# EMI-Group/evogp

Hardware: AMD Instinct MI355X
Metric: tree_evals_per_s (higher is better)
Workload: dtype f32; 1 GPU; BASELINE north_star / configs[2] shape: SymbolicRegression synthetic 10-var, GLOBAL pop=1000000 x 1024 datapoints, max_tree_len=64, funcs + - * /, one tree_SR_fitness pass over every rank's shard per step; global_pop=1000000, pop_per_gpu=1000000, datapoints=1024, var_len=10, max_tree_len=64, ranks=1, device_prewarm_calls=40

## Files before the change

evogp_amd/_lib.py:

```python
from __future__ import annotations

import ctypes as C
import os

_HERE = os.path.dirname(os.path.abspath(__file__))
LIB_PATH = os.environ.get("EVOGP_HIP_LIB") or os.path.join(_HERE, "lib", "libevogp_hip.so")

ABI_VERSION = 9

_vp = C.c_void_p
_u = C.c_uint
_i = C.c_int
_f = C.c_float

PROTOTYPES = {
    "evogp_hip_generate": [_u, _u, _u, _u, _u, _f, _f, _vp, _vp, _vp, _vp, _vp, _vp, _vp, _u, _vp],
    "evogp_hip_mutate": [_i, _i, _vp, _vp, _vp, _vp, _vp, _vp, _vp, _vp, _vp, _vp, _vp],
    "evogp_hip_crossover": [_i, _i, _i, _vp, _vp, _vp, _vp, _vp, _vp, _vp, _vp, _vp, _vp, _vp],
    "evogp_hip_evaluate": [_u, _u, _u, _u, _vp, _vp, _vp, _vp, _vp, _vp],
    "evogp_hip_sr_fitness": [_u, _u, _u, _u, _u, _i, _vp, _vp, _vp, _vp, _vp, _vp, _u, _vp],
    "evogp_hip_generate_masked": [_u, _u, _u, _u, _u, _f, _f, _vp, _vp, _vp, _vp, _vp, _vp, _vp, _u, _vp, _u, _vp],
    "evogp_hip_breed_default": [_i, _i, _i, _i, _vp, _vp, _vp, _vp, _vp, _u, _vp, _vp, _vp, _vp, _vp, _vp, _vp, _vp],
    "evogp_hip_breed_default_rows": [_i, _i, _i, _i, _vp, _vp, _vp, _vp, _vp, _u, _vp, _vp, _vp, _vp, _vp, _vp, _vp, _i, _i, _vp],
    "evogp_hip_breed_default_table": [_i, _i, _i, _i, _i, _vp, _vp, _vp, _vp, _vp, _u, _vp, _vp, _vp, _vp, _vp, _vp, _vp, _i, _i, _vp],
# ... 36 lines not shown
    "evogp_hip_tree_classes": [_u, _u, _vp, _vp, _vp, _vp, _vp, _vp, _vp],
    "evogp_hip_sr_linear_scaling": [_u, _u, _u, _u, _u, _vp, _vp, _vp, _vp, _vp, _vp, _vp, _vp],
    "evogp_hip_wrap_linear": [_u, _u, _u, _vp, _vp, _vp, _vp, _vp, _vp, _vp, _vp, _vp],
    "evogp_hip_tree_intervals": [_u, _u, _u, _vp, _vp, _vp, _vp, _vp, _vp, _vp, _vp, _vp],
    "evogp_hip_tree_derivative_intervals": [_u, _u, _u, _vp, _vp, _vp, _vp, _vp, _u, _vp, _vp, _vp, _vp, _vp, _vp, _vp, _vp],
}

DEBUG_PROTOTYPES = {
    "evogp_hip_timer_begin": [_vp],
    "evogp_hip_timer_end": [_vp, C.POINTER(C.c_float)],
    "evogp_hip_debug_set_stats": [_vp],
    "evogp_hip_debug_compile_batch": [_i],
    "evogp_hip_debug_long_compiler": [_i],
    "evogp_hip_debug_twins": [_i],
    "evogp_hip_debug_tc_fold": [_i],
    "evogp_hip_debug_profile": [_i],
    "evogp_hip_debug_profile_read": [C.POINTER(C.c_float), C.POINTER(C.c_int)],
    "evogp_hip_debug_tc_histogram": [_u, _vp, _i, _vp],
    "evogp_hip_debug_tc_nhandlers": [],
    "evogp_hip_debug_tc_program": [_u, _vp, _i],
    "evogp_hip_debug_forget_function_classes": [],
    "evogp_hip_debug_structural_mutate_given": [_i, _i, _i, _i, _i, _vp, _vp, _vp, _vp, _vp, _vp, _vp, _vp],
    "evogp_hip_debug_insert_mutate_given": [_i, _i, _i, _vp, _vp, _vp, _vp, _vp, _vp, _vp, _vp, _vp, _vp, _vp],
    "evogp_hip_debug_point_mutate_given": [_i, _i, _i, _i, _i, _i, _i, _i, _i, _vp, _vp, _vp, _vp, _vp, _vp, _vp, _vp, _vp, _vp, _vp, _vp, _vp, _vp],
    "evogp_hip_debug_lexicase": [_vp, _i],
    "evogp_hip_debug_pareto_rank": [_i],
}


def _load() -> C.CDLL:
# ... 34 lines not shown
```

evogp_amd/csrc/gen/gen_tc_asm.py:

```python
#!/usr/bin/env python3
import os
import sys

sys.path.insert(0, os.path.dirname(os.path.abspath(__file__)))
from ocml_bodies import BODIES
from pair_rows import Pairing, check as check_pairing

FORMS = ("SS", "SV", "VS", "SC", "CS", "VV", "VC", "CV")
SENTINEL_HEAVY = 0x7FC0FEED
OPS = ("add", "sub", "mul", "div")
UNARY = ("neg", "abs", "sin", "cos", "tan", "sqrt", "lsqrt", "exp", "log", "llog")
GBIN = ("ldiv", "max", "min", "lt", "gt", "le", "ge", "pow", "lpow")
GUN = ("zero", "sinh", "cosh", "tanh", "one", "rcp")
HEAVY_REGS = 24
SLOT = 256
DIVIP_REGS = 12
DIVIP = ("SS", "SC", "CS")
DIVR = ("SV", "VV", "CV")
NOPF_TWINS = tuple(f"{op}_{form}" for op in ("add", "sub", "mul") for form in FORMS) + ("push_c", "push_v") \
    + tuple(f"divip_{f}" for f in DIVIP) + tuple(f"divr_{f}" for f in DIVR)
NHF = 37 + 2 * len(UNARY) + 8 + 2 + 4 + len(DIVIP) + 1 + 1 + len(DIVR) + len(NOPF_TWINS) + 1


NOPF = False
SPLAT = False
FMA_LOSS = False
PKARITH = True
DIVABREAST = True
PKCONST = True
TRUST = True
DIVFIX = False
DIVRANGE = True
DIV_LO, DIV_HI = 0x28800000, 0x56800000
EARLYREC = True
L2WARM = True
KWARM_LINES = 4
# ... 99 lines not shown
        hid[f"{uop}_S"], hid[f"{uop}_V"] = 36 + 2 * u, 37 + 2 * u
    hid["next"] = 36 + 2 * len(UNARY)
    nh = hid["next"] + 1
    for f, form in enumerate(FORMS):
        hid[f"gbin_{form}"] = nh + f
    hid["gun_S"], hid["gun_V"], hid["if_sss"], hid["acc_s"], hid["mo_begin"], hid["end_mo"] = (nh + 8 + i for i in range(6))
    for i, form in enumerate(DIVIP):
        hid[f"divip_{form}"] = nh + 14 + i
    hid["end_cls"] = nh + 14 + len(DIVIP)
    hid["swap"] = nh + 14 + len(DIVIP) + 1
    for i, form in enumerate(DIVR):
        hid[f"divr_{form}"] = nh + 14 + len(DIVIP) + 2 + i
    for i, name in enumerate(NOPF_TWINS):
        hid[name + "_np"] = nh + 14 + len(DIVIP) + 2 + len(DIVR) + i
    hid["nan_tree"] = nh + 14 + len(DIVIP) + 2 + len(DIVR) + len(NOPF_TWINS)
    assert NHF == hid["nan_tree"] + 1 and 2 * NHF * SLOT <= 65536
    twin = [False]

    A_REC, A_WORK, A_TREES, A_DISP, A_START, A_TICK = NV - 1, NV - 2, NV - 3, NV - 4, NV - 5, NV - 6

    def tick_begin():
        if stats:
            a(f"s_memtime s[{T1}:{T2}]")
            a("s_waitcnt lgkmcnt(0)")
            a(f"v_mov_b32 v{A_TICK}, s{T1}")

    def tick_end(acc):
        if stats:
            a(f"s_memtime s[{T1}:{T2}]")
            a("s_waitcnt lgkmcnt(0)")
            a(f"v_sub_u32 v{A_TICK}, s{T1}, v{A_TICK}")
# ... 866 lines not shown
        for op in ("add", "sub", "mul"):
            for form in FORMS:
                arith(op, form, fl)
        push_c()
        push_v()
        divip_stubs()
        divr_stubs()
        twin[0] = False
        begin("nan_tree", fl)
        a("s_set_gpr_idx_off")
        a(f"s_mov_b32 s{T1}, 0x7fc00000")
        a(f"s_mov_b32 m0, s{sB}")
        a(f"s_bitset1_b64 s[{sOK}:{sOK + 1}], s{sB}")
        a(f"v_writelane_b32 v7, s{T1}, m0")
        a(f"s_branch {lab('next_tree')}")
    a(f".org {lab('hbase')}+{SLOT * 2 * NHF}")

    ALLREL = MODE["SRC0"] | MODE["SRC1"] | MODE["SRC2"] | MODE["DST"]
    for fl in (0, 1):
        for form in DIVIP:
            a(f"{lab(f'divip_body_{form}{fl}')}:")
            nops = 2 if form == "SS" else 1
            m0_stack(ALLREL, -nops * K)
            tb = S0 + nops * K
            tmp = [tb + i for i in range(DIVIP_REGS)]
            q, acc = tmp[4], tmp[0]
            if form == "SS":
                xs, ys = [S0 + K + k for k in range(K)], [S0 + k for k in range(K)]
            elif form == "CS":
                xs, ys = [f"s{sA}"] * K, [S0 + k for k in range(K)]
# ... 1202 lines not shown
```

evogp_amd/csrc/sr_tc.hip:

```cpp
#include "interp.hpp"
#include "launch.hpp"
#include "sr_params.hpp"
#include "tc_interp_k8.inc"
#include "tc_interp_k4.inc"
#include "tc_interp_k1.inc"

#include <atomic>
#include <cstddef>
#include <mutex>
#include <cstdio>
#include <vector>

namespace evogp {

struct TcCompileParams {
    const float *value;
    const int16_t *type;
    const int16_t *size;
    uint2 *prog;
    float *fitness;
    unsigned *marks;
    unsigned *zero_next;
    int pop, gp_len, var_len;
    uint32_t unary_mask;
// ... 2 lines not shown
    uint32_t rec;
    uint32_t overflow;
    int depth;
    int out_len;
    int nblocks;
    int rows;
    int general;
    int heavy_reserve;
    int div_reserve;
    int classify;
    uint32_t recip;
    int twins;
    int long_fast;
    int learn;
    int nan_trees;
};

__device__ inline uint32_t division_in_place(uint32_t id, int after, const TcCompileParams &p) {
    if (id < 24u || id >= 32u) return id;
    const uint32_t form = id - 24u;
    const uint32_t ip = form == 0u ? (uint32_t)EVOGP_TC_H_DIVIP_SS : form == 3u ? (uint32_t)EVOGP_TC_H_DIVIP_SC : form == 4u ? (uint32_t)EVOGP_TC_H_DIVIP_CS : 0u;
    if (ip == 0u) return id;
    const int before = after + (form == 0u ? 1 : 0);
    return before + p.div_reserve <= p.depth ? ip : id;
}

enum : int { TC_S = 0, TC_V = 1, TC_C = 2 };
constexpr int kMarkSampleBlocks = 64;
constexpr int kZeroRounds = 3;
static std::atomic<int> g_long_fast{-1};
static std::atomic<int> g_twins{-1};
static std::atomic<int> g_fold{-1};
static std::atomic<int> g_compile_batch{-2};
static int tc_nan_trees() {
    static const int env_fold = env_int("EVOGP_TC_FOLD", 2);
    const int fo = g_fold.load(std::memory_order_relaxed);
    return fo >= 0 ? fo : (env_fold < 0 || env_fold > 2 ? 2 : env_fold);
}
static_assert(kSentinelHeavy == 0x7FC0FEEDu, "gen/gen_tc_asm.py SENTINEL_HEAVY");

__device__ inline float fold_bin4_fast(int op, float x, float y) {
    return op == 0 ? x + y : op == 1 ? x - y : op == 2 ? x * y : (y == 0.0f ? __builtin_nanf("") : x / y);
}

__device__ inline uint32_t tc_word0(int id, int slot, uint32_t pf_bytes, uint32_t aux = 0u) {
    return ((pf_bytes >> 10) << 24) | ((aux & 0xFFu) << 16) | (uint32_t)(((slot & 1) * EVOGP_TC_NHANDLERS + id) * EVOGP_TC_SLOT);
}
// ... 260 lines not shown
    const int hf = seli(kept, totf - (inclf - deltaf), 0);
    if (any(hf > p.depth)) return p.gp_len > 64 && p.general ? TREE_GENERAL : TREE_HEAVY;
    const int dform = id - 24;
    const int ip = seli(dform == 0, (int)EVOGP_TC_H_DIVIP_SS, seli(dform == 3, (int)EVOGP_TC_H_DIVIP_SC, seli(dform == 4, (int)EVOGP_TC_H_DIVIP_CS, 0)));
    const bool inplace = (ip != 0) & (hf + (int)(dform == 0) + p.div_reserve <= p.depth);
    id = seli(inplace, ip, id);
    if (p.twins)
        id += seli(next_word_has_variable(p, keptmask, kept, !pushc & seli(isB, lV | rV, kind == 0), is_root), 0,
                   no_prefetch_delta(isB & !pushc & !divr & (opx < 3), pushc, inplace, divr & !pushc));
    if (kept) rec[slot] = make_uint2(tc_word0(id, slot, pf, aux), d1);
    if (lane == 0) rec[n] = make_uint2(tc_word0(EVOGP_TC_H_END, n, p.ydelta), 0u);
    return TREE_OK;
}


template <bool U0>
__device__ inline int compile_pack_arith(const TcCompileParams &p, char *rec0, uint32_t roff, unsigned long long inm, int lo, int len, int ty, int sz, float val, int lane) {
    typedef unsigned long long M;
    auto bperm = [](int v, int i4) -> int { return __builtin_amdgcn_ds_bpermute(i4, v); };
    auto next = [](int v) -> int { return __builtin_amdgcn_update_dpp(0, v, 0x130 , 0xf, 0xf, true); };
    auto B = [](bool c) -> M { return __builtin_amdgcn_ballot_w64(c); };
    auto L = [](M m) -> bool { return __builtin_amdgcn_inverse_ballot_w64(m); };
    auto seli = [](bool c, int x, int y) -> int { return c ? x : y; };
    auto selu = [](bool c, uint32_t x, uint32_t y) -> uint32_t { return c ? x : y; };
    auto self = [](bool c, float x, float y) -> float { return c ? x : y; };
    const M Min = inm;
    const int end = lo + len;
    asm volatile("" : "+v"(ty), "+v"(val));
    const uint32_t f = (uint32_t)val;
    const M MV = B(ty == T_VAR), MC = B(ty == T_CONST), MBf = B(ty == T_BFUNC);
    const uint32_t opu = f - (uint32_t)F_ADD;
    const M M4 = MBf & B(opu < 4u);
// ... 114 lines not shown
        cls = seg_any(Min & B(kind == 3)) ? TREE_HEAVY : seg_any(Min & B(kind == 5)) ? TREE_GENERAL : seg_any(Min & Msb) ? TREE_HEAVY
            : seg_any(Min & Mhigh) ? (p.gp_len > 64 && p.general ? TREE_GENERAL : TREE_HEAVY) : seg_any(Mlong) ? TREE_HEAVY : TREE_OK;
    }
    const M Mdivown = MB & ~Mpushc & ~Mdivr & B(opx == 3);
    const M Mss = Mdivown & B(form == 0), Msc = Mdivown & B(form == 3), Mcs = Mdivown & B(form == 4);
    const int ip = seli(L(Mss), (int)EVOGP_TC_H_DIVIP_SS, seli(L(Msc), (int)EVOGP_TC_H_DIVIP_SC, (int)EVOGP_TC_H_DIVIP_CS));
    const M Minpl = (Mss | Msc | Mcs) & B(hf + seli(L(Mss), 1, 0) + p.div_reserve <= p.depth);
    id = seli(L(Minpl), ip, id);
    if (p.twins) {
        const M Muses = ~Mpushc & ~MU & ((MB & (MlV | MrV)) | (~MB & MV));
        const M Uk = Mkept & Muses;
        const M nxt = (((~keptwave) + (Uk << 1)) & keptwave) | Mroot;
        id += seli(L(nxt), 0, no_prefetch_delta(L(MB & ~Mpushc & ~Mdivr & B(opx < 3)), L(Mpushc), L(Minpl), L(Mdivr & ~Mpushc)));
    }
    const M Mok = B(cls == TREE_OK);
    if (L(Mkept & Mok & ~Mpz)) *(uint2 *)(rec0 + (roff + (uint32_t)slot * 8u)) = make_uint2(tc_word0(id, slot, pf, aux), d1);
    if (L(Mroot)) {
        uint32_t skip = tc_word0(EVOGP_TC_H_SKIP, 0, 0u), nan_tree = tc_word0(EVOGP_TC_H_NAN_TREE, 0, 0u);
        asm volatile("" : "+v"(skip), "+v"(nan_tree));
        const uint32_t last = selu(L(Mpz), nan_tree, tc_word0(EVOGP_TC_H_END, slot + 1, p.ydelta));
        *(uint2 *)(rec0 + (roff + (uint32_t)seli(L(Mok & ~Mpz), slot + 1, 0) * 8u)) = make_uint2(selu(L(Mok), last, skip), 0u);
    }
    if (cls == TREE_GENERAL && !p.general) cls = TREE_HEAVY;
    return L(Min) ? cls : (int)TREE_OK;
}

template <bool U0>
__device__ inline int compile_pack_arith_plain(const TcCompileParams &p, char *rec0, uint32_t roff, bool in, int lo, int len, int ty, int sz, float val, int lane) {
    auto bperm = [](int v, int i4) -> int { return __builtin_amdgcn_ds_bpermute(i4, v); };
    auto next = [](int v) -> int { return __builtin_amdgcn_update_dpp(0, v, 0x130 , 0xf, 0xf, true); };
    auto any = [](bool c) -> bool { return __builtin_amdgcn_ballot_w64(c) != 0ull; };
    auto seli = [](bool c, int x, int y) -> int { return c ? x : y; };
    auto selu = [](bool c, uint32_t x, uint32_t y) -> uint32_t { return c ? x : y; };
    auto self = [](bool c, float x, float y) -> float { return c ? x : y; };
    const int end = lo + len;
    const uint32_t f = (uint32_t)val;
// ... 1104 lines not shown
    const uint32_t f = (uint32_t)val;
    return (ty == T_TFUNC) | ((ty == T_BFUNC) & (f - (uint32_t)F_ADD >= 4u)) | ((ty == T_UFUNC) & ((f == (uint32_t)F_LOOSE_INV) | (f - (uint32_t)F_SINH <= 2u)));
}

template <int B, int MODE, bool LONGROWS>
__global__ __launch_bounds__(256) void tc_compile_packed_kernel(TcCompileParams p) {
    constexpr bool UN = MODE != 0;
    const int lane = threadIdx.x & 63;
    if (p.zero_next && blockIdx.x == 0)
        for (int i = threadIdx.x; i < kCallScratchWords; i += blockDim.x) p.zero_next[i] = 0u;
    const uint32_t wave_id = uni((blockIdx.x * blockDim.x + threadIdx.x) >> 6);
    const uint32_t t0 = wave_id * (uint32_t)B;
    if (t0 >= (uint32_t)p.pop) return;
    const int nb = (int)min((uint32_t)B, (uint32_t)p.pop - t0);
    const int L = p.gp_len;
    int raw = 1;
    if (lane < nb) raw = (int)p.size[(size_t)(t0 + (uint32_t)lane) * L];
    char *const rec0 = (char *)p.prog + (size_t)t0 * p.rec;
    const bool longer = LONGROWS && lane < nb && min(raw, L) > 64;
    if (LONGROWS && longer) {
        uint32_t skip = tc_word0(EVOGP_TC_H_SKIP, 0, 0u);
        asm volatile("" : "+v"(skip));
        *(uint2 *)(rec0 + (uint32_t)__mul24(lane, (int)p.rec)) = make_uint2(skip, 0u);
        p.fitness[t0 + (uint32_t)lane] = bits2f(p.general ? kSentinelGeneral : kSentinelHeavy);
        if (p.marks) {
            if (p.general) {
                const int n = min(raw, L);
                p.marks[p.long_fast ? 8 + (int)(n > 128) + (int)(n > 256) + (int)(n > 512) : 4] = 1u;
            }
            else {
// ... 47 lines not shown
    uint32_t seen = 0u;
    while (more) {
        const bool in = n_in;
        const unsigned long long inm = n_inm;
        const int tb = n_tb, lo = n_lo, len = n_len, bad = n_bad, sz = n_sz;
        const int ty = bad ? -1 : n_ty;
        const float val = n_val;
        more = left != 0ull;
        if (more) plan();
        const uint32_t roff = (uint32_t)__mul24(tb, (int)p.rec);
        int cls;
        const bool unary = __builtin_amdgcn_ballot_w64(ty == T_UFUNC) != 0ull;
        if (MODE == 3) cls = compile_pack_mo(p, rec0, roff, in, lo, len, ty, sz, val, lane);
        else if (MODE == 2 && __builtin_amdgcn_ballot_w64(generic_node(ty, val)) != 0ull) cls = compile_pack_generic(p, rec0, roff, in, lo, len, ty, sz, val, lane);
        else if (UN && unary && p.unary_mask != 0u) cls = compile_pack_unary<true>(p, rec0, roff, in, lo, len, ty, sz, val, lane);
        else if (!UN && unary) cls = compile_pack_arith<true>(p, rec0, roff, inm, lo, len, ty, sz, val, lane);
        else cls = compile_pack_arith<false>(p, rec0, roff, inm, lo, len, ty, sz, val, lane);
        if (MODE != 3 && p.learn) {
            const bool look = MODE != 0 || __builtin_amdgcn_ballot_w64(cls != TREE_OK) != 0ull;
            if (look) {
                const bool gen = __builtin_amdgcn_ballot_w64(generic_node(ty, val)) != 0ull;
                const bool un = unary && __builtin_amdgcn_ballot_w64((ty == T_UFUNC) & ((uint32_t)val - (uint32_t)F_SIN <= (uint32_t)(F_LOOSE_SQRT - F_SIN))) != 0ull;
                seen |= ((un | gen) ? 1u : 0u) | (gen ? 2u : 0u);
            }
        }
        if (cls != TREE_OK && in && lane == lo) {
            const bool nan = bad != 0 || cls == TREE_BAD;
            p.fitness[t0 + (uint32_t)tb] = nan ? __builtin_nanf("") : bits2f(cls == TREE_GENERAL ? kSentinelGeneral : kSentinelHeavy);
            if (!nan && p.marks) {
                if (cls == TREE_GENERAL) p.marks[p.long_fast ? 8 : 4] = 1u;
                else {
                    p.marks[0] = 1u;
// ... 733 lines not shown
        st_trees += nb; st_batches += 1u;
#endif
        t0 = t0n; nb = nbn;
    }
#ifdef EVOGP_FUSED_STATS
    if (p.t.stats && lane == 0) {
        unsigned long long *s = p.t.stats;
        atomicAdd(s + 0, (unsigned long long)st_first); atomicAdd(s + 1, (unsigned long long)st_comp); atomicAdd(s + 2, (unsigned long long)st_grab);
        atomicAdd(s + 3, (unsigned long long)st_asm); atomicAdd(s + 4, (unsigned long long)st_trees); atomicAdd(s + 5, (unsigned long long)st_batches);
        atomicAdd(s + 6, (unsigned long long)(clock64() - st_begin)); atomicAdd(s + 7, 1ull);
        atomicAdd(s + 8, (unsigned long long)st_cp); atomicAdd(s + 9, (unsigned long long)st_plan);
    }
#endif
}

namespace {

struct TcDevice {
    std::mutex mu;
    void *prog = nullptr;
    size_t prog_bytes = 0;
    void *graph_prog = nullptr;
    size_t graph_bytes = 0;
    std::vector<void *> retired;
    size_t retired_bytes = 0;
    hipEvent_t last_use = nullptr;
    hipStream_t last_stream = nullptr;
    bool last_use_pending = false;
    bool multi_stream = false;
    unsigned char attr_set[24] = {};
    hipStream_t side = nullptr;
    hipEvent_t fork = nullptr, ready[kCallScratchChunks] = {};
    int last_pop = 0;
    const char *last_records = nullptr;
    uint32_t last_rec = 0, last_overflow = 0;
    struct Ring { hipStream_t stream; void *buf; };
    std::vector<Ring> rings;
    void *spare_ring = nullptr;
    size_t ring_bytes = 0;
    static constexpr int kFbSlots = 8;
    unsigned *fb_host = nullptr, *fb_dev = nullptr;
    struct FbKey { int pop, gp_len; unsigned long long stamp; } fb_key[kFbSlots] = {};
    unsigned long long fb_clock = 0;
};

TcDevice g_tc[64];

static hipError_t order_behind_last_use(TcDevice &d, hipStream_t stream) {
    if (d.last_stream == stream || (!d.last_use_pending && !d.last_use)) return hipSuccess;
    hipError_t e;
// ... 112 lines not shown
        if ((e = order_behind_last_use(d, stream)) != hipSuccess) return e;
        if (need_buf > d.prog_bytes) {
            if (d.prog) {
                if ((e = hipDeviceSynchronize()) != hipSuccess) return e;
                engine_free(d.prog);
                d.prog = nullptr; d.prog_bytes = 0;
            }
            const size_t cap = need_buf + need / 8;
            if ((e = engine_alloc(&d.prog, cap)) != hipSuccess) return e;
            d.prog_bytes = cap;
        }
        records = (char *)d.prog;
    }
    if (!d.last_use && (e = hipEventCreateWithFlags(&d.last_use, hipEventDisableTiming)) != hipSuccess) return e;
    d.last_pop = p.pop; d.last_rec = rec; d.last_overflow = (uint32_t)overflow;

    int chunks = 1;
    static const int env_chunks = env_int("EVOGP_TC_CHUNKS", 0);
    if (p.marks && !capturing && !STATS && !p.prof_mid && pieces == 1) {
        if (env_chunks > 0) chunks = env_chunks;
        if (chunks > kCallScratchChunks) chunks = kCallScratchChunks;
        if (chunks > 1 && p.pop / chunks < 20000) chunks = p.pop / 20000 > 0 ? p.pop / 20000 : 1;
    }
    if (chunks > 1) {
        if (!d.side && (e = hipStreamCreateWithFlags(&d.side, hipStreamNonBlocking)) != hipSuccess) return e;
        if (!d.fork && (e = hipEventCreateWithFlags(&d.fork, hipEventDisableTiming)) != hipSuccess) return e;
        for (int i = 0; i < chunks; ++i)
            if (!d.ready[i] && (e = hipEventCreateWithFlags(&d.ready[i], hipEventDisableTiming)) != hipSuccess) return e;
        if (wg_waves * 2 > waves_per_cu) wg_waves = waves_per_cu / 2 > 0 ? waves_per_cu / 2 : 1;
        wgs_per_cu = 1;
// ... 18 lines not shown
        c.out_len = p.out_len; c.nblocks = nblocks; c.rows = K;
        c.heavy_reserve = (EVOGP_TC_HEAVY_REGS + K - 1) / K;
        c.div_reserve = env_divip ? (EVOGP_TC_DIVIP_REGS + K - 1) / K : 1 << 20;
        c.classify = p.classify;
        c.recip = recip ? (uint32_t)(p.var_len + label_cols) * c.var_stride : 0u;
        {
            static const int env_twins = env_int("EVOGP_TC_TWINS", 1);
            const int tw = g_twins.load(std::memory_order_relaxed);
            c.twins = tw >= 0 ? tw : (env_twins == 2 || (env_twins == 1 && (long)n >= 900l * info.num_cus));
        }
        c.general = env_general != 0;
        { const int lf = g_long_fast.load(std::memory_order_relaxed); c.long_fast = (lf >= 0 ? lf : env_long_fast) && p.out_len == 1 && p.gp_len >= 128 && c.general; }
        c.unary_mask = (uint32_t)env_unary & ((uint32_t)EVOGP_TC_UNARY_MASK | (1u << kUnaryInv));
        c.learn = p.feedback != nullptr && marks != nullptr;
        c.nan_trees = tc_nan_trees();
        return c;
    };
    bool learn_packed = false;
    auto launch_marked_general = [&](const TcCompileParams &c, int n, hipStream_t strm) {
        long gblocks = ((long)n + 63) / 64;
        if (gblocks > (long)info.num_cus * 16) gblocks = (long)info.num_cus * 16;
        if (p.gp_len <= 64) { hipLaunchKernelGGL(tc_compile_general_kernel<false>, dim3((unsigned)gblocks), dim3(256), 0, strm, c, 0, 0, p.gp_len); return; }
        if (c.long_fast && c.general && c.gp_len >= 128) {
            if (4 * tc_long_lds_bytes(c.gp_len) > 64 * 1024 && !d.attr_set[16]) {
                (void)hipFuncSetAttribute((const void *)tc_compile_long_kernel, hipFuncAttributeMaxDynamicSharedMemorySize, 160 * 1024 - 1024);
                (void)hipGetLastError();
                d.attr_set[16] = true;
            }
            int lo_len = 0, klass = 0;
            for (int hi_len = 128; ; hi_len *= 2, ++klass) {
                if (hi_len > c.gp_len) hi_len = c.gp_len;
                const int group = hi_len <= 256 ? 16 : 64;
                hipLaunchKernelGGL(tc_compile_long_kernel, dim3((unsigned)((n + group - 1) / group)), dim3(256), 4 * tc_long_lds_bytes(hi_len), strm, c, lo_len, hi_len, group, klass);
                if (hi_len >= c.gp_len) break;
                lo_len = hi_len;
            }
        }
        hipLaunchKernelGGL(tc_compile_general_kernel<true>, dim3((unsigned)gblocks), dim3(256), 4 * tc_general_lds_bytes(p.gp_len), strm, c, 0, 0, p.gp_len);
    };
    auto launch_compilers = [&](int lo, int n, unsigned *marks, bool first, hipStream_t strm) -> hipError_t {
        const TcCompileParams c = compile_params(lo, n, marks, first);
        long cblocks = ((long)n + 3) / 4;
        long cmax = (long)info.num_cus * 32;
        if (env_cblocks > 0) cmax = env_cblocks;
        if (cblocks > cmax) cblocks = cmax;
        if (first) {
            const long nwaves = cblocks * 4, sw = kMarkSampleBlocks * 4 < nwaves ? kMarkSampleBlocks * 4 : nwaves;
            long sample = 0;
            for (long w = 0; w < sw && w < n; ++w) sample += (n - 1 - w) / nwaves + 1;
            *mark_sample = (int)sample;
        }
        const size_t clds = 4 * tc_general_lds_bytes(p.gp_len);
        if (clds > 64 * 1024 && !d.attr_set[15]) {
            (void)hipFuncSetAttribute((const void *)tc_compile_general_kernel<true>, hipFuncAttributeMaxDynamicSharedMemorySize, 160 * 1024 - 1024);
            (void)hipGetLastError();
            d.attr_set[15] = true;
        }
        static const int env_packed_env = env_int("EVOGP_TC_PACKED", -1);
        const int set_packed = g_compile_batch.load(std::memory_order_relaxed);
        const int env_packed = set_packed != -2 ? set_packed : env_packed_env;
        static const int env_generic = env_int("EVOGP_TC_PACK_GENERIC", 1);
        const bool packed_mo = p.out_len > 1 && env_packed != 0 && env_generic != 0;
        const bool packed = (p.out_len == 1 && env_packed != 0) || packed_mo;
        if (packed) {
            const bool un = c.nblocks != 1;
            constexpr unsigned kOwnHandlers = (1u << F_ADD) | (1u << F_SUB) | (1u << F_MUL) | (1u << F_DIV) | (1u << F_SIN) | (1u << F_COS) | (1u << F_TAN) |
                                              (1u << F_LOG) | (1u << F_LOOSE_LOG) | (1u << F_EXP) | (1u << F_INV) | (1u << F_NEG) | (1u << F_ABS) |
                                              (1u << F_SQRT) | (1u << F_LOOSE_SQRT);
            const bool may_generic = p.func_mask == 0u || (p.func_mask & ~kOwnHandlers) != 0u;
            const int mode = packed_mo ? 3 : (c.general && p.hint_general && env_generic != 0 && may_generic) ? 2 : (un || c.gp_len > 64) ? 1 : 0;
            int B = n >= 400000 ? 32 : n >= 200000 ? 16 : 8;
            if (env_packed > 0) B = env_packed >= 64 ? 64 : env_packed >= 32 ? 32 : env_packed >= 16 ? 16 : 8;
            if (mode >= 2) B = B >= 16 ? 32 : 8;
            static const int env_pwg = env_int("EVOGP_TC_PACKED_WG", 0);
            const int wgw = env_pwg == 64 ? 1 : env_pwg == 256 ? 4 : n >= 120000 ? 1 : 4;
            const long pblocks = ((long)n + wgw * B - 1) / (wgw * B);
            if (first) *mark_sample = (int)std::min<long>(n, (long)kMarkSampleBlocks * 4 * B);
            learn_packed = c.learn != 0 && mode != 3;
            const dim3 grid((unsigned)pblocks), wg(64 * wgw);
            const bool longrows = c.gp_len > 64;
#define EVOGP_LAUNCH_MODE(BB, MM) \
            do { if (longrows) hipLaunchKernelGGL((tc_compile_packed_kernel<BB, MM, true>), grid, wg, 0, strm, c); \
                 else hipLaunchKernelGGL((tc_compile_packed_kernel<BB, MM, false>), grid, wg, 0, strm, c); } while (0)
#define EVOGP_LAUNCH_PACKED(BB) \
            do { if (mode == 1) EVOGP_LAUNCH_MODE(BB, 1); \
// ... 375 lines not shown
    __shared__ unsigned h_s[2 * EVOGP_TC_NHANDLERS];
    for (int i = threadIdx.x; i < 2 * EVOGP_TC_NHANDLERS; i += blockDim.x) h_s[i] = 0u;
    __syncthreads();
    const int t = (int)(blockIdx.x * blockDim.x + threadIdx.x);
    if (t < pop) {
        const char *r = (const char *)prog + (size_t)t * rec;
        bool more = true;
        for (int blk = 0; blk < 64 && more; ++blk) {
            const uint2 *w = (const uint2 *)r;
            more = false;
            for (int i = 0; i < 32; ++i) {
                const unsigned h = (w[i].x & 0xFFFFu) / EVOGP_TC_SLOT;
                if (h >= 2u * EVOGP_TC_NHANDLERS) break;
                const unsigned id = h % EVOGP_TC_NHANDLERS;
                atomicAdd(h_s + h, 1u);
                if (id == EVOGP_TC_H_END || id == EVOGP_TC_H_END_MO || id == EVOGP_TC_H_END_CLS || id == EVOGP_TC_H_SKIP || id == EVOGP_TC_H_NAN_TREE) break;
                if (id == EVOGP_TC_H_NEXT) { r += w[i].y; more = true; break; }
            }
        }
    }
    __syncthreads();
    for (int i = threadIdx.x; i < 2 * EVOGP_TC_NHANDLERS; i += blockDim.x)
        if (h_s[i]) atomicAdd(hist + i, (unsigned long long)h_s[i]);
}

hipError_t tc_histogram(int pop, unsigned long long *hist, int hist_len, hipStream_t stream) {
    int dev = 0;
    (void)hipGetDevice(&dev);
    TcDevice &d = g_tc[dev & 63];
    std::lock_guard<std::mutex> lock(d.mu);
    if (!d.last_records || d.last_pop <= 0 || hist_len < 2 * EVOGP_TC_NHANDLERS) return hipErrorInvalidValue;
// ... 54 lines not shown

}

extern "C" int evogp_hip_debug_twins(int mode) {
    if (mode < -1 || mode > 1) return EVOGP_E_BADARG;
    evogp::g_twins.store(mode, std::memory_order_relaxed);
    return EVOGP_OK;
}

extern "C" int evogp_hip_debug_tc_fold(int mode) {
    if (mode < -1 || mode > 2) return EVOGP_E_BADARG;
    evogp::g_fold.store(mode, std::memory_order_relaxed);
    return EVOGP_OK;
}

extern "C" int evogp_hip_debug_long_compiler(int fast) {
    if (fast < -1 || fast > 1) return EVOGP_E_BADARG;
    evogp::g_long_fast.store(fast, std::memory_order_relaxed);
    return EVOGP_OK;
}

extern "C" int evogp_hip_debug_compile_batch(int trees) {
    if (trees < -1 || trees > 64) return EVOGP_E_BADARG;
    evogp::g_compile_batch.store(trees, std::memory_order_relaxed);
    return EVOGP_OK;
}

extern "C" int evogp_hip_set_program_buffer_limit(unsigned long long bytes) {
    evogp::g_prog_limit.store(bytes, std::memory_order_relaxed);
    return EVOGP_OK;
// ... 37 lines not shown
}

extern "C" int evogp_hip_release_workspaces(void) {
    int dev = 0;
    (void)hipGetDevice(&dev);
    evogp::TcDevice &d = evogp::g_tc[dev & 63];
    std::lock_guard<std::mutex> lock(d.mu);
    for (auto &k : d.fb_key) k = {};
    const bool grad_held = evogp::grad_workspaces_held(), case_held = evogp::case_workspaces_held();
    if (!d.prog && !d.graph_prog && d.rings.empty() && !d.spare_ring && d.retired.empty() && !grad_held && !case_held) return EVOGP_OK;
    hipError_t e = hipDeviceSynchronize();
    if (e != hipSuccess) return (int)e;
    if (grad_held) evogp::release_grad_workspaces(dev);
    if (case_held) evogp::release_case_workspaces(dev);
    if (d.prog) evogp::engine_free(d.prog);
    d.prog = nullptr; d.prog_bytes = 0; d.last_pop = 0; d.last_records = nullptr;
    if (d.graph_prog) evogp::engine_free(d.graph_prog);
    d.graph_prog = nullptr; d.graph_bytes = 0;
    for (void *r : d.retired) evogp::engine_free(r);
    d.retired.clear(); d.retired_bytes = 0;
    for (auto &r : d.rings) evogp::engine_free(r.buf);
    d.rings.clear();
    if (d.spare_ring) evogp::engine_free(d.spare_ring);
    d.spare_ring = nullptr;
    return (int)e;
}

extern "C" int evogp_hip_debug_tc_histogram(unsigned pop, unsigned long long *device_hist, int hist_len, evogp_stream_t stream) {
    if (!device_hist) return EVOGP_E_NULLPTR;
    return (int)evogp::tc_histogram((int)pop, device_hist, hist_len, (hipStream_t)stream);
}
// ... 5 lines not shown
    (void)hipGetDevice(&dev);
    evogp::TcDevice &d = evogp::g_tc[dev & 63];
    std::lock_guard<std::mutex> lock(d.mu);
    if (!d.last_records || (int)tree >= d.last_pop || !host_words) return -1;
    if (hipDeviceSynchronize() != hipSuccess) return -1;
    int n = 0;
    const char *r = d.last_records + (size_t)tree * d.last_rec;
    for (int blk = 0; blk < 64 && n < max_words; ++blk) {
        unsigned w[64];
        if (hipMemcpy(w, r, 256, hipMemcpyDeviceToHost) != hipSuccess) return -1;
        bool more = false;
        for (int i = 0; i < 32 && n < max_words; ++i) {
            const unsigned h = (w[2 * i] & 0xFFFFu) / EVOGP_TC_SLOT, id = h % EVOGP_TC_NHANDLERS;
            if (id == EVOGP_TC_H_NEXT && h < 2u * EVOGP_TC_NHANDLERS) { r += w[2 * i + 1]; more = true; break; }
            host_words[2 * n] = w[2 * i]; host_words[2 * n + 1] = w[2 * i + 1]; ++n;
            if (h >= 2u * EVOGP_TC_NHANDLERS || id == EVOGP_TC_H_END || id == EVOGP_TC_H_END_MO || id == EVOGP_TC_H_END_CLS || id == EVOGP_TC_H_SKIP) break;
        }
        if (!more) break;
    }
    return n;
}
```

include/evogp_hip_debug.h:

```cpp
#ifndef EVOGP_HIP_DEBUG_H
#define EVOGP_HIP_DEBUG_H
#include "evogp_hip.h"
#ifdef __cplusplus
extern "C" {
#endif

int evogp_hip_timer_begin(evogp_stream_t stream);
int evogp_hip_timer_end(evogp_stream_t stream, float *elapsed_ms);

int evogp_hip_debug_set_stats(unsigned long long *device_counters);

int evogp_hip_debug_profile(int enable);
int evogp_hip_debug_profile_read(float *stage_ms , int *calls);

int evogp_hip_debug_compile_batch(int trees);
int evogp_hip_debug_long_compiler(int fast);
int evogp_hip_debug_twins(int mode);
int evogp_hip_debug_tc_fold(int mode);

int evogp_hip_debug_tc_histogram(unsigned pop, unsigned long long *device_hist, int hist_len, evogp_stream_t stream);
int evogp_hip_debug_tc_nhandlers(void);
int evogp_hip_debug_tc_program(unsigned tree, unsigned *host_words, int max_words);

int evogp_hip_debug_forget_function_classes(void);

int evogp_hip_debug_structural_mutate_given(int pop_size, int gp_len, int mode, int inner_is_offset, int skip_rows, const int *given,
                                            const float *value, const int16_t *type, const int16_t *size, float *value_res,
                                            int16_t *type_res, int16_t *size_res, evogp_stream_t stream);
int evogp_hip_debug_insert_mutate_given(int pop_size, int gp_len, int skip_rows, const int *given, const float *value, const int16_t *type,
                                        const int16_t *size, const float *donor_value, const int16_t *donor_type, const int16_t *donor_size,
                                        float *value_res, int16_t *type_res, int16_t *size_res, evogp_stream_t stream);
int evogp_hip_debug_point_mutate_given(int pop_size, int gp_len, int mode, int modify_output, int fix_roulette, int skip_rows, int input_len,
                                       int output_len, int n_consts, const unsigned char *target, const float *u, const int *var_idx,
// ... 13 lines not shown
```

Before: 1678 billion tree-evals/s.

## Precompute fitness of single-variable leaf trees and short-circuit their evaluation

Adds a small kernel that computes, for each input variable, the total error of a tree consisting only of that variable. The compiler detects single-node variable trees and emits a new leaf_tree handler record carrying the precomputed sum, so the evaluator writes the fitness directly instead of running the tree over all datapoints. It is enabled by default for large populations and adds one extra kernel launch per compile. Whether it pays off depends on how many trees in the population are single variables.

New measurement: 1691 billion tree-evals/s, median of 6. About the same (+0.7%).

```diff
diff --git a/evogp_amd/_lib.py b/evogp_amd/_lib.py
--- a/evogp_amd/_lib.py
+++ b/evogp_amd/_lib.py
@@ -74,6 +74,8 @@
     "evogp_hip_debug_long_compiler": [_i],
     "evogp_hip_debug_twins": [_i],
     "evogp_hip_debug_tc_fold": [_i],
+    "evogp_hip_debug_tc_leaf": [_i],
+    "evogp_hip_debug_leaf_sums": [_vp, _i],
     "evogp_hip_debug_profile": [_i],
     "evogp_hip_debug_profile_read": [C.POINTER(C.c_float), C.POINTER(C.c_int)],
     "evogp_hip_debug_tc_histogram": [_u, _vp, _i, _vp],
diff --git a/evogp_amd/csrc/gen/gen_tc_asm.py b/evogp_amd/csrc/gen/gen_tc_asm.py
--- a/evogp_amd/csrc/gen/gen_tc_asm.py
+++ b/evogp_amd/csrc/gen/gen_tc_asm.py
@@ -19,7 +19,7 @@
 DIVR = ("SV", "VV", "CV")
 NOPF_TWINS = tuple(f"{op}_{form}" for op in ("add", "sub", "mul") for form in FORMS) + ("push_c", "push_v") \
     + tuple(f"divip_{f}" for f in DIVIP) + tuple(f"divr_{f}" for f in DIVR)
-NHF = 37 + 2 * len(UNARY) + 8 + 2 + 4 + len(DIVIP) + 1 + 1 + len(DIVR) + len(NOPF_TWINS) + 1
+NHF = 37 + 2 * len(UNARY) + 8 + 2 + 4 + len(DIVIP) + 1 + 1 + len(DIVR) + len(NOPF_TWINS) + 2
 
 
 NOPF = False
@@ -149,7 +149,8 @@
     for i, name in enumerate(NOPF_TWINS):
         hid[name + "_np"] = nh + 14 + len(DIVIP) + 2 + len(DIVR) + i
     hid["nan_tree"] = nh + 14 + len(DIVIP) + 2 + len(DIVR) + len(NOPF_TWINS)
-    assert NHF == hid["nan_tree"] + 1 and 2 * NHF * SLOT <= 65536
+    hid["leaf_tree"] = hid["nan_tree"] + 1
+    assert NHF == hid["leaf_tree"] + 1 and 2 * NHF * SLOT <= 65536
     twin = [False]
 
     A_REC, A_WORK, A_TREES, A_DISP, A_START, A_TICK = NV - 1, NV - 2, NV - 3, NV - 4, NV - 5, NV - 6
@@ -1046,6 +1047,13 @@
         a(f"s_bitset1_b64 s[{sOK}:{sOK + 1}], s{sB}")
         a(f"v_writelane_b32 v7, s{T1}, m0")
         a(f"s_branch {lab('next_tree')}")
+        begin("leaf_tree", fl)
+        a("s_set_gpr_idx_off")
+        a(f"s_mov_b32 s{T1}, s{W + 1}")
+        a(f"s_mov_b32 m0, s{sB}")
+        a(f"s_bitset1_b64 s[{sOK}:{sOK + 1}], s{sB}")
+        a(f"v_writelane_b32 v7, s{T1}, m0")
+        a(f"s_branch {lab('next_tree')}")
     a(f".org {lab('hbase')}+{SLOT * 2 * NHF}")
 
     ALLREL = MODE["SRC0"] | MODE["SRC1"] | MODE["SRC2"] | MODE["DST"]
diff --git a/evogp_amd/csrc/sr_tc.hip b/evogp_amd/csrc/sr_tc.hip
--- a/evogp_amd/csrc/sr_tc.hip
+++ b/evogp_amd/csrc/sr_tc.hip
@@ -40,6 +40,7 @@
     int long_fast;
     int learn;
     int nan_trees;
+    const float *leaf_sums;
 };
 
 __device__ inline uint32_t division_in_place(uint32_t id, int after, const TcCompileParams &p) {
@@ -57,6 +58,7 @@
 static std::atomic<int> g_long_fast{-1};
 static std::atomic<int> g_twins{-1};
 static std::atomic<int> g_fold{-1};
+static std::atomic<int> g_leaf{-1};
 static std::atomic<int> g_compile_batch{-2};
 static int tc_nan_trees() {
     static const int env_fold = env_int("EVOGP_TC_FOLD", 2);
@@ -347,8 +349,8 @@
 }
 
 
-template <bool U0>
-__device__ inline int compile_pack_arith(const TcCompileParams &p, char *rec0, uint32_t roff, unsigned long long inm, int lo, int len, int ty, int sz, float val, int lane) {
+template <bool U0, bool LEAF = false>
+__device__ inline int compile_pack_arith(const TcCompileParams &p, char *rec0, uint32_t roff, unsigned long long inm, int lo, int len, int ty, int sz, float val, int lane, float leaf) {
     typedef unsigned long long M;
     auto bperm = [](int v, int i4) -> int { return __builtin_amdgcn_ds_bpermute(i4, v); };
     auto next = [](int v) -> int { return __builtin_amdgcn_update_dpp(0, v, 0x130 , 0xf, 0xf, true); };
@@ -493,12 +495,21 @@
         id += seli(L(nxt), 0, no_prefetch_delta(L(MB & ~Mpushc & ~Mdivr & B(opx < 3)), L(Mpushc), L(Minpl), L(Mdivr & ~Mpushc)));
     }
     const M Mok = B(cls == TREE_OK);
-    if (L(Mkept & Mok & ~Mpz)) *(uint2 *)(rec0 + (roff + (uint32_t)slot * 8u)) = make_uint2(tc_word0(id, slot, pf, aux), d1);
+    const M Mlf = LEAF && p.leaf_sums ? Mroot & MV & Mok & B(len == 1) : 0ull;
+    uint32_t leaf_sum = 0u;
+    if (Mlf != 0ull) leaf_sum = (uint32_t)bperm((int)f2bits(leaf), v << 2);
+    if (L(Mkept & Mok & ~Mpz & ~Mlf)) *(uint2 *)(rec0 + (roff + (uint32_t)slot * 8u)) = make_uint2(tc_word0(id, slot, pf, aux), d1);
     if (L(Mroot)) {
         uint32_t skip = tc_word0(EVOGP_TC_H_SKIP, 0, 0u), nan_tree = tc_word0(EVOGP_TC_H_NAN_TREE, 0, 0u);
         asm volatile("" : "+v"(skip), "+v"(nan_tree));
-        const uint32_t last = selu(L(Mpz), nan_tree, tc_word0(EVOGP_TC_H_END, slot + 1, p.ydelta));
-        *(uint2 *)(rec0 + (roff + (uint32_t)seli(L(Mok & ~Mpz), slot + 1, 0) * 8u)) = make_uint2(selu(L(Mok), last, skip), 0u);
+        uint32_t last = selu(L(Mpz), nan_tree, tc_word0(EVOGP_TC_H_END, slot + 1, p.ydelta)), last1 = 0u;
+        if (Mlf != 0ull) {
+            uint32_t leaf_tree = tc_word0(EVOGP_TC_H_LEAF_TREE, 0, 0u);
+            asm volatile("" : "+v"(leaf_tree));
+            last = selu(L(Mlf), leaf_tree, last);
+            last1 = selu(L(Mlf), leaf_sum, 0u);
+        }
+        *(uint2 *)(rec0 + (roff + (uint32_t)seli(L(Mok & ~Mpz & ~Mlf), slot + 1, 0) * 8u)) = make_uint2(selu(L(Mok), last, skip), last1);
     }
     if (cls == TREE_GENERAL && !p.general) cls = TREE_HEAVY;
     return L(Min) ? cls : (int)TREE_OK;
@@ -1633,6 +1644,8 @@
     if (t0 >= (uint32_t)p.pop) return;
     const int nb = (int)min((uint32_t)B, (uint32_t)p.pop - t0);
     const int L = p.gp_len;
+    float leaf = 0.0f;
+    if (MODE == 0 && p.leaf_sums && lane < p.var_len) leaf = p.leaf_sums[lane];
     int raw = 1;
     if (lane < nb) raw = (int)p.size[(size_t)(t0 + (uint32_t)lane) * L];
     char *const rec0 = (char *)p.prog + (size_t)t0 * p.rec;
@@ -1710,8 +1723,8 @@
         if (MODE == 3) cls = compile_pack_mo(p, rec0, roff, in, lo, len, ty, sz, val, lane);
         else if (MODE == 2 && __builtin_amdgcn_ballot_w64(generic_node(ty, val)) != 0ull) cls = compile_pack_generic(p, rec0, roff, in, lo, len, ty, sz, val, lane);
         else if (UN && unary && p.unary_mask != 0u) cls = compile_pack_unary<true>(p, rec0, roff, in, lo, len, ty, sz, val, lane);
-        else if (!UN && unary) cls = compile_pack_arith<true>(p, rec0, roff, inm, lo, len, ty, sz, val, lane);
-        else cls = compile_pack_arith<false>(p, rec0, roff, inm, lo, len, ty, sz, val, lane);
+        else if (!UN && unary) cls = compile_pack_arith<true, MODE == 0>(p, rec0, roff, inm, lo, len, ty, sz, val, lane, leaf);
+        else cls = compile_pack_arith<false, MODE == 0>(p, rec0, roff, inm, lo, len, ty, sz, val, lane, leaf);
         if (MODE != 3 && p.learn) {
             const bool look = MODE != 0 || __builtin_amdgcn_ballot_w64(cls != TREE_OK) != 0ull;
             if (look) {
@@ -2475,6 +2488,42 @@
 #endif
 }
 
+template <int CTRL, int ROWS, bool ZERO_FILL>
+__device__ inline float leaf_dpp_add(float acc, int lane) {
+    const float moved = bits2f((uint32_t)__builtin_amdgcn_update_dpp(0, (int)f2bits(acc), CTRL, ROWS, 0xf, ZERO_FILL));
+    const float sum = moved + acc;
+    return ((ROWS >> (lane >> 4)) & 1) ? sum : acc;
+}
+template <int K>
+__global__ __launch_bounds__(64) void leaf_sums_kernel(const float *X, const float *y, int D, int var_len, int mse, float *leaf_sums) {
+    constexpr int RPL = K < 4 ? K : 4;
+    const int lane = (int)threadIdx.x, j = (int)blockIdx.x;
+    const int tiles = (D + 64 * K - 1) / (64 * K);
+    float acc = 0.0f;
+    for (int tile = 0; tile < tiles; ++tile) {
+        float e[K];
+#pragma unroll
+        for (int k = 0; k < K; ++k) {
+            const int row = tile * 64 * K + (k >> 2) * 256 + RPL * lane + (k & 3), at = min(row, D - 1);
+            const float d = y[at] - X[(size_t)at * (size_t)var_len + (size_t)j];
+            const float q = mse ? d * d : fabsf(d);
+            e[k] = row < D ? q : 0.0f;
+        }
+#pragma unroll
+        for (int k = 0; k < K; ++k) acc += e[k];
+    }
+    acc = leaf_dpp_add<0x111, 0xf, true>(acc, lane);
+    acc = leaf_dpp_add<0x112, 0xf, true>(acc, lane);
+    acc = leaf_dpp_add<0x114, 0xf, true>(acc, lane);
+    acc = leaf_dpp_add<0x118, 0xf, true>(acc, lane);
+    acc = leaf_dpp_add<0x142, 0xa, false>(acc, lane);
+    acc = leaf_dpp_add<0x143, 0xc, false>(acc, lane);
+    if (lane == 63) {
+        const uint32_t w = f2bits(acc);
+        leaf_sums[j] = bits2f((w & 0x7FFFFFFFu) > 0x7F800000u ? 0x7FC00000u : w);
+    }
+}
+
 namespace {
 
 struct TcDevice {
@@ -2495,6 +2544,8 @@
     int last_pop = 0;
     const char *last_records = nullptr;
     uint32_t last_rec = 0, last_overflow = 0;
+    const float *last_leaf_sums = nullptr;
+    int last_leaf_vars = 0;
     struct Ring { hipStream_t stream; void *buf; };
     std::vector<Ring> rings;
     void *spare_ring = nullptr;
@@ -2637,6 +2688,7 @@
     }
     if (!d.last_use && (e = hipEventCreateWithFlags(&d.last_use, hipEventDisableTiming)) != hipSuccess) return e;
     d.last_pop = p.pop; d.last_rec = rec; d.last_overflow = (uint32_t)overflow;
+    d.last_leaf_sums = nullptr; d.last_leaf_vars = 0;
 
     int chunks = 1;
     static const int env_chunks = env_int("EVOGP_TC_CHUNKS", 0);
@@ -2685,8 +2737,13 @@
         c.unary_mask = (uint32_t)env_unary & ((uint32_t)EVOGP_TC_UNARY_MASK | (1u << kUnaryInv));
         c.learn = p.feedback != nullptr && marks != nullptr;
         c.nan_trees = tc_nan_trees();
+        c.leaf_sums = nullptr;
         return c;
     };
+    constexpr long kLeafMinTrees = 400000;
+    static const int env_leaf = env_int("EVOGP_TC_LEAF", 1);
+    const bool leaf_can = p.out_len == 1 && !p.classify && pieces == 1 && tc_nan_trees() >= 1 && p.var_len >= 1 && p.var_len <= 64;
+    float *const leaf_table = (float *)(records + need + 7 * (size_t)rec);
     bool learn_packed = false;
     auto launch_marked_general = [&](const TcCompileParams &c, int n, hipStream_t strm) {
         long gblocks = ((long)n + 63) / 64;
@@ -2710,7 +2767,7 @@
         hipLaunchKernelGGL(tc_compile_general_kernel<true>, dim3((unsigned)gblocks), dim3(256), 4 * tc_general_lds_bytes(p.gp_len), strm, c, 0, 0, p.gp_len);
     };
     auto launch_compilers = [&](int lo, int n, unsigned *marks, bool first, hipStream_t strm) -> hipError_t {
-        const TcCompileParams c = compile_params(lo, n, marks, first);
+        TcCompileParams c = compile_params(lo, n, marks, first);
         long cblocks = ((long)n + 3) / 4;
         long cmax = (long)info.num_cus * 32;
         if (env_cblocks > 0) cmax = env_cblocks;
@@ -2740,6 +2797,14 @@
                                               (1u << F_SQRT) | (1u << F_LOOSE_SQRT);
             const bool may_generic = p.func_mask == 0u || (p.func_mask & ~kOwnHandlers) != 0u;
             const int mode = packed_mo ? 3 : (c.general && p.hint_general && env_generic != 0 && may_generic) ? 2 : (un || c.gp_len > 64) ? 1 : 0;
+            if (mode == 0 && leaf_can && chunks == 1) {
+                const int lf = g_leaf.load(std::memory_order_relaxed);
+                if (lf >= 0 ? lf != 0 : (env_leaf == 2 || (env_leaf == 1 && (long)n >= kLeafMinTrees))) {
+                    hipLaunchKernelGGL(leaf_sums_kernel<K>, dim3((unsigned)p.var_len), dim3(64), 0, strm, p.X, p.y, p.D, p.var_len, p.use_mse ? 1 : 0, leaf_table);
+                    c.leaf_sums = leaf_table;
+                    d.last_leaf_sums = leaf_table; d.last_leaf_vars = p.var_len;
+                }
+            }
             int B = n >= 400000 ? 32 : n >= 200000 ? 16 : 8;
             if (env_packed > 0) B = env_packed >= 64 ? 64 : env_packed >= 32 ? 32 : env_packed >= 16 ? 16 : 8;
             if (mode >= 2) B = B >= 16 ? 32 : 8;
@@ -3145,7 +3210,8 @@
                 if (h >= 2u * EVOGP_TC_NHANDLERS) break;
                 const unsigned id = h % EVOGP_TC_NHANDLERS;
                 atomicAdd(h_s + h, 1u);
-                if (id == EVOGP_TC_H_END || id == EVOGP_TC_H_END_MO || id == EVOGP_TC_H_END_CLS || id == EVOGP_TC_H_SKIP || id == EVOGP_TC_H_NAN_TREE) break;
+                if (id == EVOGP_TC_H_END || id == EVOGP_TC_H_END_MO || id == EVOGP_TC_H_END_CLS || id == EVOGP_TC_H_SKIP || id == EVOGP_TC_H_NAN_TREE ||
+                    id == EVOGP_TC_H_LEAF_TREE) break;
                 if (id == EVOGP_TC_H_NEXT) { r += w[i].y; more = true; break; }
             }
         }
@@ -3230,6 +3296,25 @@
     return EVOGP_OK;
 }
 
+extern "C" int evogp_hip_debug_tc_leaf(int mode) {
+    if (mode < -1 || mode > 1) return EVOGP_E_BADARG;
+    evogp::g_leaf.store(mode, std::memory_order_relaxed);
+    return EVOGP_OK;
+}
+
+extern "C" int evogp_hip_debug_leaf_sums(float *host_sums, int n) {
+    int dev = 0;
+    (void)hipGetDevice(&dev);
+    evogp::TcDevice &d = evogp::g_tc[dev & 63];
+    std::lock_guard<std::mutex> lock(d.mu);
+    if (!d.last_leaf_sums) return 0;
+    if (!host_sums || n < 0) return -1;
+    if (hipDeviceSynchronize() != hipSuccess) return -1;
+    const int m = n < d.last_leaf_vars ? n : d.last_leaf_vars;
+    if (m > 0 && hipMemcpy(host_sums, d.last_leaf_sums, (size_t)m * sizeof(float), hipMemcpyDeviceToHost) != hipSuccess) return -1;
+    return d.last_leaf_vars;
+}
+
 extern "C" int evogp_hip_debug_long_compiler(int fast) {
     if (fast < -1 || fast > 1) return EVOGP_E_BADARG;
     evogp::g_long_fast.store(fast, std::memory_order_relaxed);
@@ -3297,7 +3382,7 @@
     if (grad_held) evogp::release_grad_workspaces(dev);
     if (case_held) evogp::release_case_workspaces(dev);
     if (d.prog) evogp::engine_free(d.prog);
-    d.prog = nullptr; d.prog_bytes = 0; d.last_pop = 0; d.last_records = nullptr;
+    d.prog = nullptr; d.prog_bytes = 0; d.last_pop = 0; d.last_records = nullptr; d.last_leaf_sums = nullptr; d.last_leaf_vars = 0;
     if (d.graph_prog) evogp::engine_free(d.graph_prog);
     d.graph_prog = nullptr; d.graph_bytes = 0;
     for (void *r : d.retired) evogp::engine_free(r);
@@ -3333,7 +3418,8 @@
             const unsigned h = (w[2 * i] & 0xFFFFu) / EVOGP_TC_SLOT, id = h % EVOGP_TC_NHANDLERS;
             if (id == EVOGP_TC_H_NEXT && h < 2u * EVOGP_TC_NHANDLERS) { r += w[2 * i + 1]; more = true; break; }
             host_words[2 * n] = w[2 * i]; host_words[2 * n + 1] = w[2 * i + 1]; ++n;
-            if (h >= 2u * EVOGP_TC_NHANDLERS || id == EVOGP_TC_H_END || id == EVOGP_TC_H_END_MO || id == EVOGP_TC_H_END_CLS || id == EVOGP_TC_H_SKIP) break;
+            if (h >= 2u * EVOGP_TC_NHANDLERS || id == EVOGP_TC_H_END || id == EVOGP_TC_H_END_MO || id == EVOGP_TC_H_END_CLS || id == EVOGP_TC_H_SKIP ||
+                id == EVOGP_TC_H_NAN_TREE || id == EVOGP_TC_H_LEAF_TREE) break;
         }
         if (!more) break;
     }
diff --git a/include/evogp_hip_debug.h b/include/evogp_hip_debug.h
--- a/include/evogp_hip_debug.h
+++ b/include/evogp_hip_debug.h
@@ -17,6 +17,8 @@
 int evogp_hip_debug_long_compiler(int fast);
 int evogp_hip_debug_twins(int mode);
 int evogp_hip_debug_tc_fold(int mode);
+int evogp_hip_debug_tc_leaf(int mode);
+int evogp_hip_debug_leaf_sums(float *host_sums, int n);
 
 int evogp_hip_debug_tc_histogram(unsigned pop, unsigned long long *device_hist, int hist_len, evogp_stream_t stream);
 int evogp_hip_debug_tc_nhandlers(void);
```
